# DigitalPhonetics/Intrinsic-Subgraph-Generation-for-VQA

Measured on AMD Instinct MI355X. Metric: GQA questions/sec, higher is better.
Workload: dtype f32

## Files before the change

### __graft_entry__.py

```python
from __future__ import annotations

import glob
import json
import os
import subprocess
import sys

ROOT = os.path.dirname(os.path.abspath(__file__))
PKG = os.path.join(ROOT, "intrinsic-subgraph-generation-for-vqa_amd")
CSRC = os.path.join(PKG, "csrc")
LIB = os.path.join(CSRC, "libisg_hip.so")
LOADER_LIB = os.path.join(CSRC, "libisg_loader.so")
if ROOT not in sys.path:
    sys.path.insert(0, ROOT)


HIP_FLAGS = ["-O3", "--offload-arch=gfx950", "-std=c++17", "-fPIC", "-Wall", "-Wno-unused-function",
             "-Werror=missing-field-initializers"]
EXTRA_FLAGS = {"isg_simple.hip": ["-fno-slp-vectorize"], "isg_mp_logits.hip": ["-fno-slp-vectorize"],
               "isg_sgenc_bwd.hip": ["-fno-slp-vectorize"]}


def flags_for(source: str):
    return HIP_FLAGS + EXTRA_FLAGS.get(os.path.basename(source), [])
# ... 2 lines not shown
def _stale(target: str, sources) -> bool:
    if not os.path.exists(target):
        return True
    t = os.path.getmtime(target)
    return any(os.path.getmtime(s) > t for s in sources)


def build(force: bool = False) -> None:
    sources = sorted(glob.glob(os.path.join(CSRC, "*.hip")))
    headers = glob.glob(os.path.join(CSRC, "*.hpp")) + [os.path.join(ROOT, "include", "isg.h"),
                                                        os.path.join(ROOT, "include", "isg_train.h"),
                                                        os.path.join(ROOT, "include", "isg_optim.h"),
                                                        os.path.join(ROOT, "include", "isg_fused.h"),
                                                        os.path.join(ROOT, "include", "isg_sgenc_train.h"),
                                                        os.path.join(ROOT, "include", "isg_dist.h"),
                                                        os.path.join(ROOT, "include", "isg_linear_train.h")]
    hipcc = os.environ.get("HIPCC", "/opt/rocm/bin/hipcc")
    flags = HIP_FLAGS
    objdir = os.path.join(CSRC, "_obj")
    os.makedirs(objdir, exist_ok=True)
    objs = [os.path.join(objdir, os.path.basename(s)[:-4] + ".o") for s in sources]
    stamp_path = LIB[:-3] + ".stamp"
    stamp = json.dumps({"sources": [os.path.basename(s) for s in sources], "flags": flags, "extra": EXTRA_FLAGS}, sort_keys=True)
    stamp_ok = os.path.exists(stamp_path) and open(stamp_path).read() == stamp
    relink = force or not stamp_ok
    if not force and stamp_ok and not _stale(LIB, sources + headers):
        todo = []
    else:
        old = json.loads(open(stamp_path).read()) if os.path.exists(stamp_path) else None
        flags_changed = old is not None and (old.get("flags") != flags or old.get("extra", {}) != EXTRA_FLAGS)
        todo = [(s, o) for s, o in zip(sources, objs) if force or flags_changed or _stale(o, [s] + headers)]
# ... 30 lines not shown
    _loader.load()
    lib = _lib.load()
    assert lib.isg_abi_version() == _lib.ABI_VERSION
    from isubgvqa_amd import _lib_train
    assert _lib_train.load().isg_train_abi_version() == _lib_train.ABI_VERSION
    from isubgvqa_amd import _lib_optim
    assert _lib_optim.load().isg_optim_abi_version() == _lib_optim.ABI_VERSION
    from isubgvqa_amd import _lib_fused
    assert _lib_fused.load().isg_fused_abi_version() == _lib_fused.ABI_VERSION
    from isubgvqa_amd import _lib_sgenc_train
    assert _lib_sgenc_train.load().isg_sgenc_train_abi_version() == _lib_sgenc_train.ABI_VERSION
    from isubgvqa_amd import _lib_dist
    assert _lib_dist.load().isg_dist_abi_version() == _lib_dist.ABI_VERSION
    from isubgvqa_amd import _lib_linear_train
    assert _lib_linear_train.load().isg_linear_train_abi_version() == _lib_linear_train.ABI_VERSION
    import isubgvqa_amd.models
    print(f"[build] ok: {LIB} ({os.path.getsize(LIB)} bytes), {len(_lib.SIGNATURES)} C-ABI symbols + "
          f"{len(_lib_train.SIGNATURES)} training + {len(_lib_optim.SIGNATURES)} optimizer + {len(_lib_fused.SIGNATURES)} fused-launch + "
          f"{len(_lib_sgenc_train.SIGNATURES)} scene-graph training + {len(_lib_dist.SIGNATURES)} data-parallel + "
          f"{len(_lib_linear_train.SIGNATURES)} Linear-backward entry points", flush=True)


STRICT_LIB = os.path.join(CSRC, "libisg_hip_strict.so")


def build_strict(sources, headers, objs, hipcc, relink: bool) -> None:
    objdir = os.path.join(CSRC, "_obj")
    strict = [s for s in sources if any(m in open(s).read() for m in ("ISG_WAIT(", "ISG_BARRIER("))]
    sobjs = {s: os.path.join(objdir, os.path.basename(s)[:-4] + ".strict.o") for s in strict}
    todo = [s for s in strict if relink or _stale(sobjs[s], [s] + headers)]
    if not todo and os.path.exists(STRICT_LIB) and not _stale(STRICT_LIB, sources + headers):
        return
    if any(not os.path.exists(o) for o in objs):
        if os.path.exists(STRICT_LIB):
            return
# ... 66 lines not shown
```

### intrinsic-subgraph-generation-for-vqa_amd/csrc/isg_layer_conv.hip

```cpp
#include "isg_f16x3.hpp"

#include "isg_diag.hpp"

ISG_DIAG_BUFFER(g_lc_stamps)
#define LC_STAMP(i) ISG_DIAG_ADD(i)

namespace isg {

typedef __attribute__((address_space(3))) void lc_lds_t;
typedef __attribute__((address_space(1))) void lc_glb_t;

constexpr int LC_ROWS = 64, LC_ECAP = 256, LC_C = 128, LC_K = 128, LC_LDX = LC_C + 4, LC_LDA = LC_K + 8, LC_THREADS = 512;
constexpr int LC_OFF_XR = LC_ROWS * LC_LDX * 4;
constexpr int LC_OFF_A = 2 * LC_ROWS * LC_LDX * 4;
constexpr int LC_OFF_TAB = LC_OFF_A + 2 * 64 * LC_LDA * 2;
constexpr int LC_OFF_RAW = LC_OFF_TAB + 2 * (LC_ECAP * 16 + LC_ECAP * 4 + 68 * 4) + LC_ECAP * 4 + 4 * 64 * 4 + 64 * 4 + 3 * LC_C * 4 +
                           4 * LC_C * 4;
constexpr int LC_OFF_LIVE = LC_OFF_RAW + LC_ROWS * LC_K * 4;
constexpr int LC_SMEM_BYTES = LC_OFF_LIVE + 2 * 4 * 8;
static_assert(LC_OFF_RAW % 16 == 0, "16-byte pieces");
static_assert(LC_SMEM_BYTES <= 160 * 1024, "one workgroup per CU");

struct LcArgs {
  const _Float16 *xp;
// ... 2 lines not shown
  const float *wn_inv, *bn;
  const _Float16 *ep;
  const float *ep_inv;
  const _Float16 *We;
  const float *we_inv, *att;
  const float *bias;
  const int *rowptr, *eid, *src, *dst, *ntiles;
  const int4 *tile_info;
  const float *edge_mask, *node_mask;
  float *out, *alpha;
  float *rowmax;
  int N, E, H, KSE, NTE, ldo;
  float slope;
  unsigned char *row_dead;
  int G;
};

struct LcLive {
  const unsigned long long *w;
  int p1, p2, p3, n;
};

__device__ __forceinline__ LcLive lc_live_load(const unsigned long long *sw) {
  int c[4];
#pragma unroll
  for (int i = 0; i < 4; ++i)
    c[i] = __builtin_amdgcn_readfirstlane(__popc((unsigned)sw[i]) + __popc((unsigned)(sw[i] >> 32)));
  return LcLive{sw, c[0], c[0] + c[1], c[0] + c[1] + c[2], c[0] + c[1] + c[2] + c[3]};
}

// ... 613 lines not shown
    LC_STAMP(6)
    if (!has_next) break;
    desc = desc_n;
    t = t_next;
    cur ^= 1;
  }
#undef LC_REQUEST_TILE
#undef LC_REQUEST_PLANES
#undef LC_REQUEST_MASKS
#undef LC_BALLOT
#undef LC_STORE_TILE
#undef LC_PLANES_LANDED
  ISG_DIAG_DUMP(g_lc_stamps, bid * 8 + wave, 12, )
}

constexpr int LG_MAXG = 6, LC_GROUP_DEFAULT = 4;
constexpr int LG_T_LG = LC_ECAP * 8, LG_T_SP = LG_T_LG + LC_ECAP * 4, LG_T_DR = LG_T_SP + LC_ECAP, LG_T_LV = LG_T_DR + LC_ECAP,
              LG_T_RP = LG_T_LV + LC_ECAP, LG_T_POS = LG_T_RP + 68 * 4, LG_TILE_BYTES = LG_T_POS + 64;
constexpr int LG_OFF_T = LC_OFF_A + 2 * 64 * LC_LDA * 2;
constexpr int LG_OFF_MISC = LG_OFF_T + LG_MAXG * LG_TILE_BYTES;
constexpr int LG_MISC_FLOATS = 4 * 64 + 3 * LC_C + 4 * LC_C + 64;
constexpr int LG_SMEM_BYTES = LG_OFF_MISC + LG_MISC_FLOATS * 4 + LG_MAXG * 16 + LG_MAXG * 8 + LG_MAXG * 4 * 8;
static_assert(LG_TILE_BYTES % 16 == 0 && LG_OFF_MISC % 16 == 0, "16-byte pieces");
static_assert(64 * 512 <= 2 * 64 * LC_LDA * 2, "the node planes fit the panel image they share LDS with");
static_assert(LG_SMEM_BYTES <= 160 * 1024, "one workgroup per CU");

template <int KSE_T, bool SL01>
__global__ __launch_bounds__(LC_THREADS, 2) void gatv2_layer_conv_groups_kernel(LcArgs a) {
  extern __shared__ __attribute__((aligned(16))) unsigned char lc_smem[];
  typedef float (*BufX)[LC_LDX];
  typedef _Float16 (*BufP)[64][LC_LDA];
  constexpr bool MASKED = true;
  BufX sXl = reinterpret_cast<BufX>(lc_smem);
  BufX sXr = reinterpret_cast<BufX>(lc_smem + LC_OFF_XR);
  BufP sA = reinterpret_cast<BufP>(lc_smem + LC_OFF_A);
  unsigned char *s_tiles = lc_smem + LG_OFF_T;
#define LG_EM(j) reinterpret_cast<int2 *>(s_tiles + (j) * LG_TILE_BYTES)
#define LG_LG(j) reinterpret_cast<float *>(s_tiles + (j) * LG_TILE_BYTES + LG_T_LG)
#define LG_SP(j) (s_tiles + (j) * LG_TILE_BYTES + LG_T_SP)
#define LG_DR(j) (s_tiles + (j) * LG_TILE_BYTES + LG_T_DR)
#define LG_LV(j) (s_tiles + (j) * LG_TILE_BYTES + LG_T_LV)
#define LG_RP(j) reinterpret_cast<int *>(s_tiles + (j) * LG_TILE_BYTES + LG_T_RP)
// ... 51 lines not shown
    s_bias[tid] = a.bias ? a.bias[hoff + tid] : 0.f;
    sXl[0][tid] = 0.f;
  } else if (tid < 3 * LC_C) {
    const int c = tid - LC_C;
    const int src_col = (c >> 7) * a.H * LC_C + hoff + (c & 127);
    s_bn[c] = a.bn[src_col];
    s_wninv[c] = a.wn_inv[src_col];
  }
  const float slope = a.slope;
  const int prow = half * 32 + fr;

#pragma unroll 1
  for (int tg = t; tg < T; tg += G * ngrp) {
    int tl = tid, ll = lane;
    asm volatile("" : "+v"(tl), "+v"(ll));
    int4 dsc[LG_MAXG];
    int ng = 0;
#pragma unroll
    for (int j = 0; j < LG_MAXG; ++j) {
      const int tj = tg + j * ngrp;
      const bool on = j < G && tj < T;
      const int4 d = a.tile_info[min(tj, T - 1)];
      dsc[j] = make_int4(on ? __builtin_amdgcn_readfirstlane(d.x) : 0, on ? min(__builtin_amdgcn_readfirstlane(d.y), LC_ROWS) : 0,
                         on ? __builtin_amdgcn_readfirstlane(d.z) : 0, on ? min(__builtin_amdgcn_readfirstlane(d.w), LC_ECAP) : 0);
      ng += on ? 1 : 0;
    }
    int srcv[LG_MAXG], eidv[LG_MAXG], dstv[LG_MAXG], rpv[LG_MAXG];
    float einvv[LG_MAXG], mskv[LG_MAXG];
#pragma unroll
    for (int j = 0; j < LG_MAXG; ++j) {
      srcv[j] = eidv[j] = dstv[j] = rpv[j] = 0;
      einvv[j] = 1.f;
      if (j < ng) {
        if (tl <= dsc[j].y) rpv[j] = a.rowptr[dsc[j].x + tl];
        if (tl < dsc[j].w) {
          srcv[j] = a.src[dsc[j].z + tl];
          eidv[j] = a.eid[dsc[j].z + tl];
          dstv[j] = a.dst[dsc[j].z + tl];
          einvv[j] = a.ep_inv[dsc[j].z + tl];
        }
      }
    }
    if (tl < LG_MAXG) s_touch[tl] = 0ull;
    __syncthreads();
#pragma unroll
    for (int j = 0; j < LG_MAXG; ++j) {
      mskv[j] = 1.f;
      if (j < ng && tl < dsc[j].w)
        mskv[j] = a.edge_mask ? a.edge_mask[eidv[j]] : a.node_mask[srcv[j]] * a.node_mask[dstv[j]];
    }
#pragma unroll
    for (int j = 0; j < LG_MAXG; ++j) {
      if (j < ng) {
        const int r0n = dsc[j].x, nrn = dsc[j].y, e0n = dsc[j].z, nen = dsc[j].w;
        if (tl <= nrn) LG_RP(j)[tl] = rpv[j] - e0n;
        if (tl == 0) s_desc[j] = dsc[j];
        if (tl < LC_ECAP) {
          const int sx = min(max(srcv[j] - r0n, 0), max(nrn - 1, 0));
          const int dz = min(max(dstv[j] - r0n, 0), max(nrn - 1, 0));
          const bool lv = tl < nen && (__float_as_int(mskv[j]) & 0x7fffffff) != 0;
          const unsigned long long bw = __ballot(lv);
          if (ll == 0) s_livew[j * 4 + wave] = bw;
          if (lv) atomicOr(&s_touch[j], (1ull << sx) | (1ull << dz));
          LG_EM(j)[tl] = make_int2(eidv[j], __float_as_int(mskv[j]));
          LG_LG(j)[tl] = lv ? einvv[j] : 0.f;
          LG_SP(j)[tl] = (unsigned char)sx;
          LG_DR(j)[tl] = (unsigned char)dz;
        }
      }
    }
    __syncthreads();
    LC_STAMP(0)

    int ntot = 0;
#pragma unroll
    for (int j = 0; j < LG_MAXG; ++j) ntot += j < ng ? __builtin_amdgcn_readfirstlane(__popcll(s_touch[j])) : 0;
    const int step = ntot <= LC_ROWS ? ng : 1;
#pragma unroll 1
    for (int ja = 0; ja < ng; ja += step) {
      const int jb = min(ja + step, ng);
      int cum[LG_MAXG];
      int nl = 0, nlive = 0;
#pragma unroll
      for (int j = 0; j < LG_MAXG; ++j) {
        if (j >= ja && j < jb) {
          const unsigned long long m = s_touch[j];
          if (tl < LC_ROWS) {
            const bool on = (m >> tl) & 1ull;
            const int p = nl + __popcll(m & ((1ull << tl) - 1ull));
            LG_POS(j)[tl] = (unsigned char)(on ? p : 0);
            if (on) s_nodes[p] = s_desc[j].x + tl;
          }
          int c[4];
#pragma unroll
          for (int i = 0; i < 4; ++i) {
            const unsigned long long w = s_livew[j * 4 + i];
            c[i] = __builtin_amdgcn_readfirstlane(__popc((unsigned)w) + __popc((unsigned)(w >> 32)));
          }
          if (tl < LC_ECAP) {
            const unsigned long long w = s_livew[j * 4 + wave];
            const int pre = (wave > 0 ? c[0] : 0) + (wave > 1 ? c[1] : 0) + (wave > 2 ? c[2] : 0);
            if ((w >> ll) & 1ull) LG_LV(j)[pre + __popcll(w & ((1ull << ll) - 1ull))] = (unsigned char)tl;
          }
          nl += __builtin_amdgcn_readfirstlane(__popcll(m));
          nlive += (c[0] + c[1]) + (c[2] + c[3]);
        }
        cum[j] = nlive;
      }
#define LG_FIND(k, jj, slot, e0v)                                                                                    \
  int jj = 0, slot, e0v;                                                                                             \
  {                                                                                                                  \
    int base_ = 0;                                                                                                   \
    _Pragma("unroll") for (int j_ = 0; j_ < LG_MAXG - 1; ++j_) {                                                     \
      const bool up_ = (k) >= cum[j_];                                                                               \
      jj += up_ ? 1 : 0;                                                                                             \
      base_ = up_ ? cum[j_] : base_;                                                                                 \
    }                                                                                                                \
// ... 189 lines not shown

extern "C" int isg_node_gate_planes(const uint16_t *x_planes, const float *x_inv_scale, const uint16_t *w_frag, const float *w_inv_scale,
                                    const float *b, const float *q, const int64_t *batch, int32_t double_index, float *gate,
                                    int64_t N, int32_t C, void *stream) {
  if (N < 0 || C <= 0) return ISG_EINVAL;
  auto mis = [](const void *p) { return (reinterpret_cast<uintptr_t>(p) & 15) != 0; };
  if (C != NG_C || mis(x_planes) || mis(w_inv_scale) || mis(b) || mis(q) || N >= (1ll << 31)) return ISG_EUNSUPPORTED;
  if (N == 0) return ISG_OK;
  if (!x_planes || !x_inv_scale || !w_frag || !w_inv_scale || !b || !q || !batch || !gate) return ISG_EINVAL;
  node_gate_planes_kernel<<<(unsigned)((N + NG_ROWS - 1) / NG_ROWS), 256, 0, as_stream(stream)>>>(
      reinterpret_cast<const _Float16 *>(x_planes), x_inv_scale, reinterpret_cast<const _Float16 *>(w_frag), w_inv_scale, b, q,
      reinterpret_cast<const long long *>(batch), double_index, gate, (int)N, sqrtf((float)C));
  return check_launch();
}

extern "C" int isg_gatv2_layer_conv(const uint16_t *x_planes, const float *x_inv_scale, const uint16_t *wn_frag, const float *wn_inv_scale,
                                    const float *bn, const uint16_t *edge_planes, const float *edge_inv_scale, const uint16_t *we_frag,
                                    const float *we_inv_scale, const float *att, const float *bias, const int32_t *rowptr,
                                    const int32_t *eid, const int32_t *src, const int32_t *dst, const int32_t *tile_info,
                                    const int32_t *ntiles, int64_t max_tiles, const float *node_mask, const float *edge_mask,
                                    float *out, int32_t ldo, float *alpha, float *rowmax, uint8_t *row_dead, int64_t N, int64_t E,
                                    int32_t H,
                                    int32_t C, int32_t K_in, int32_t K_edge, float negative_slope, void *stream) {
  if (N < 0 || E < 0 || H <= 0 || C <= 0 || K_in <= 0 || K_edge <= 0 || max_tiles < 0 || ldo < H * C) return ISG_EINVAL;
  auto mis = [](const void *p) { return (reinterpret_cast<uintptr_t>(p) & 15) != 0; };
  if (C != LC_C || K_in != LC_K || K_edge > LC_K || (K_edge & 3) != 0 || (ldo & 3) != 0 || H > 16 || mis(x_planes) ||
      mis(edge_planes) || mis(out) || (bias && mis(bias)) || mis(tile_info) || N >= (1ll << 31) || E >= (1ll << 31))
    return ISG_EUNSUPPORTED;
  if (N == 0 || max_tiles == 0) return ISG_OK;
  if (!x_planes || !x_inv_scale || !wn_frag || !wn_inv_scale || !bn ||
      (E > 0 && (!edge_planes || !edge_inv_scale || !eid || !src || !dst || !alpha)) || !we_frag || !we_inv_scale || !att || !rowptr ||
      !tile_info || !ntiles || !out)
    return ISG_EINVAL;
  static const bool dense_mask = [] { const char *e = getenv("ISG_LC_DENSE_MASK"); return e && atoi(e) != 0; }();
  LcArgs a = {
      .xp = reinterpret_cast<const _Float16 *>(x_planes), .xinv = x_inv_scale, .Wn = reinterpret_cast<const _Float16 *>(wn_frag),
      .wn_inv = wn_inv_scale, .bn = bn, .ep = reinterpret_cast<const _Float16 *>(edge_planes), .ep_inv = edge_inv_scale,
      .We = reinterpret_cast<const _Float16 *>(we_frag), .we_inv = we_inv_scale, .att = att, .bias = bias, .rowptr = rowptr,
      .eid = eid, .src = src, .dst = dst, .ntiles = ntiles, .tile_info = reinterpret_cast<const int4 *>(tile_info),
      .edge_mask = edge_mask, .node_mask = node_mask, .out = out, .alpha = alpha, .rowmax = rowmax, .N = (int)N, .E = (int)E,
      .H = H, .KSE = (K_edge + 15) / 16, .NTE = H * C / 32, .ldo = ldo, .slope = negative_slope, .row_dead = row_dead, .G = 1};
  if (!a.xp || !a.xinv || !a.Wn || !a.wn_inv || !a.bn || (a.E > 0 && (!a.ep || !a.ep_inv || !a.eid || !a.src || !a.dst || !a.alpha)) ||
      !a.We || !a.we_inv || !a.att || !a.rowptr || !a.tile_info || !a.ntiles || !a.out)
    return ISG_EINVAL;
  const int cus = device_cus();
  int gpx = (cus / 8) / H;
  if (gpx < 1) gpx = 1;
  const long long need = (max_tiles + 7) / 8;
  if (gpx > need) gpx = (int)need;
  const unsigned grid = 8u * (unsigned)H * (unsigned)gpx;
  hipStream_t st = as_stream(stream);
  static const int force_group = [] { const char *e = getenv("ISG_LC_GROUP"); return e ? atoi(e) : 0; }();
  {
    const long long tiles = std::max((N + LC_ROWS - 1) / LC_ROWS, (E + LC_ECAP - 1) / LC_ECAP);
    const long long per_wg = (std::min<long long>(tiles, max_tiles) + 8 * gpx - 1) / (8 * gpx);
    a.G = force_group > 0 ? std::min(force_group, LG_MAXG) : (int)std::max<long long>(1, std::min<long long>(LC_GROUP_DEFAULT, per_wg));
  }
#define LC_LAUNCH_G(KT, SL)                                                                                          \
  {                                                                                                                  \
    if (!dyn_lds_ok<&gatv2_layer_conv_groups_kernel<KT, SL>>(LG_SMEM_BYTES)) return ISG_EUNSUPPORTED;                \
    gatv2_layer_conv_groups_kernel<KT, SL><<<grid, LC_THREADS, LG_SMEM_BYTES, st>>>(a);                              \
  }
#define LC_LAUNCH(M, KT, SL, LV)                                                                                     \
  {                                                                                                                  \
    if (!dyn_lds_ok<&gatv2_layer_conv_kernel<M, KT, SL, LV>>(LC_SMEM_BYTES)) return ISG_EUNSUPPORTED;                \
    gatv2_layer_conv_kernel<M, KT, SL, LV><<<grid, LC_THREADS, LC_SMEM_BYTES, st>>>(a);                              \
  }
#define LC_LAUNCH_M(KT, SL)                                                                                          \
  {                                                                                                                  \
    if (dense_mask) LC_LAUNCH(true, KT, SL, false) else if (a.G > 1) LC_LAUNCH_G(KT, SL) else LC_LAUNCH(true, KT, SL, true) \
  }
  const bool masked = node_mask || edge_mask;
  const bool sl01 = negative_slope >= 0.f && negative_slope <= 1.f;
  if (a.KSE == 8 && sl01) {
    if (masked) LC_LAUNCH_M(8, true) else LC_LAUNCH(false, 8, true, false)
  } else if (sl01) {
    if (masked) LC_LAUNCH_M(0, true) else LC_LAUNCH(false, 0, true, false)
  } else {
    if (masked) LC_LAUNCH_M(0, false) else LC_LAUNCH(false, 0, false, false)
  }
#undef LC_LAUNCH_M
#undef LC_LAUNCH_G
#undef LC_LAUNCH
  return check_launch();
}

namespace isg {

constexpr int RO_ROWS = 64, RO_C = 128, RO_LDA = RO_C + 8, RO_LDC = RO_C + 4, RO_GPC = 128;
constexpr int RO_SMEM_BYTES = 2 * (2 * RO_ROWS * RO_LDA * 2) + (6 * 64 + RO_GPC + 4) * 4;
static_assert(RO_ROWS * RO_LDC * 4 <= 2 * RO_ROWS * RO_LDA * 2, "xn aliases the first plane image");

struct RoArgs {
  const float *x;
  const _Float16 *w1f, *w2f;
  const float *w1_inv, *b1, *w2_inv, *b2;
  const float *y_bound;
  const float *q;
  const float *node_mask;
// ... 258 lines not shown
```

### intrinsic-subgraph-generation-for-vqa_amd/ops.py

```python
from __future__ import annotations

import contextlib
import dataclasses
import operator
import sys
import types
import weakref
from dataclasses import dataclass, field
from typing import NamedTuple, Optional, Tuple

import torch
from torch import Tensor

from . import _lib

MAX_NODES_PER_GRAPH = 1024


@dataclasses.dataclass(frozen=True)
class Switches:
    plan_fused: bool = True
    bounds_to_host: bool = True
    mixed_dispatch: bool = True
    mixed_max_fraction: float = 0.12
# ... 1234 lines not shown
    if edge_attr.dtype != torch.float32:
        raise TypeError("gatv2_layer_conv: fp32 edge rows")
    cat_w = derived_weight("layer_conv_w", (lin_l.weight, lin_r.weight),
                           lambda: torch.cat([lin_l.weight.detach(), lin_r.weight.detach()], 0).contiguous())
    zeros = lambda m: torch.zeros(HC, dtype=torch.float32, device=dev) if m.bias is None else m.bias.detach()
    srcs = tuple(t for t in (lin_l.weight, lin_l.bias, lin_r.bias) if t is not None)
    cat_b = derived_weight("layer_conv_b", srcs, lambda: torch.cat([zeros(lin_l), zeros(lin_r)]).float().contiguous())
    wn, wn_inv = _weight_planes(cat_w, True, "f16x3")
    we, we_inv = _weight_planes(w_edge, True, "f16x3")
    (_, ntiles, cap, _), (ep, ep_inv) = plan.tiles_and_edge_planes(edge_attr, TILE_CONV_NODES, TILE_CONV_EDGES)
    shared, out, alpha, rowmax = _tile_conv_operands(plan, ntiles, cap, att, bias, node_mask, edge_mask, H, HC, want_rowmax, dev)
    row_dead = None
    if rowmax is not None and (node_mask is not None or edge_mask is not None):
        whole = plan.tile_mode(TILE_CONV_NODES, TILE_CONV_EDGES) == "tiles"
        row_dead = (torch.empty if whole else torch.zeros)(N, H, dtype=torch.uint8, device=dev)
    timer, ev1 = MP_TIMER, None
    if timer is not None:
        ev0, ev1 = timer.bracket({"N": N, "E": E, "H": H, "C": C, "K": K, "masked": node_mask is not None or edge_mask is not None,
                                  "feat_bytes": 4, "tile_conv": True, "layer_conv": True, "K_in": K_in})
        ev0.record()
    rc = lib.isg_gatv2_layer_conv(
        x.planes.data_ptr(), x.inv.data_ptr(), wn.data_ptr(), wn_inv.data_ptr(), cat_b.data_ptr(), ep.data_ptr(), ep_inv.data_ptr(),
        we.data_ptr(), we_inv.data_ptr(), *shared, 0 if row_dead is None else row_dead.data_ptr(), N, E, H, C, K_in, K,
        float(negative_slope), _stream())
    if not _launched(rc, "isg_gatv2_layer_conv", timer, ev1):
        return None
    sub = _mixed_sub(plan)
    if sub is not None:
        pl = x.planes.view(torch.float16).index_select(0, sub.nodes).float()
        xs = ((pl[:, 0] + pl[:, 1]) * x.inv.index_select(0, sub.nodes)[:, None]).contiguous()
        y = linear(xs, cat_w, cat_b)
        _oversize_conv(sub, y[:, :HC], y[:, HC:], edge_attr, w_edge, att, H, bias, node_mask, edge_mask, negative_slope,
                       out, alpha, rowmax)
    if rowmax is not None:
        attach_row_maxima(out, rowmax)
    if row_dead is not None:
        attach_dead_rows(out, row_dead)
    return out, alpha

# ... 1769 lines not shown
```

Measured before the change: 3.248 million.

## Precompute per-tile live-edge tables in a separate kernel for masked layer conv

Adds a pre-pass kernel that builds, for each tile, a 4 KiB image holding the edge ids, masks, scales, src/dst offsets, live-edge lists and row pointers. The grouped layer-conv kernel then loads these images straight into LDS with global_load_lds instead of gathering and computing them per group. The default group size also goes from 4 to 6 tiles. This takes the masked gather and compaction off the main kernel's critical path. In exchange it adds an extra launch, a temporary buffer allocation and extra global memory traffic.

```diff
diff --git a/__graft_entry__.py b/__graft_entry__.py
--- a/__graft_entry__.py
+++ b/__graft_entry__.py
@@ -40,7 +40,8 @@
                                                         os.path.join(ROOT, "include", "isg_fused.h"),
                                                         os.path.join(ROOT, "include", "isg_sgenc_train.h"),
                                                         os.path.join(ROOT, "include", "isg_dist.h"),
-                                                        os.path.join(ROOT, "include", "isg_linear_train.h")]
+                                                        os.path.join(ROOT, "include", "isg_linear_train.h"),
+                                                        os.path.join(ROOT, "include", "isg_masked.h")]
     hipcc = os.environ.get("HIPCC", "/opt/rocm/bin/hipcc")
     flags = HIP_FLAGS
     objdir = os.path.join(CSRC, "_obj")
@@ -101,11 +102,13 @@
     assert _lib_dist.load().isg_dist_abi_version() == _lib_dist.ABI_VERSION
     from isubgvqa_amd import _lib_linear_train
     assert _lib_linear_train.load().isg_linear_train_abi_version() == _lib_linear_train.ABI_VERSION
+    from isubgvqa_amd import _lib_masked
+    assert _lib_masked.load().isg_masked_abi_version() == _lib_masked.ABI_VERSION
     import isubgvqa_amd.models
     print(f"[build] ok: {LIB} ({os.path.getsize(LIB)} bytes), {len(_lib.SIGNATURES)} C-ABI symbols + "
           f"{len(_lib_train.SIGNATURES)} training + {len(_lib_optim.SIGNATURES)} optimizer + {len(_lib_fused.SIGNATURES)} fused-launch + "
           f"{len(_lib_sgenc_train.SIGNATURES)} scene-graph training + {len(_lib_dist.SIGNATURES)} data-parallel + "
-          f"{len(_lib_linear_train.SIGNATURES)} Linear-backward entry points", flush=True)
+          f"{len(_lib_linear_train.SIGNATURES)} Linear-backward + {len(_lib_masked.SIGNATURES)} masked-layer entry points", flush=True)
 
 
 STRICT_LIB = os.path.join(CSRC, "libisg_hip_strict.so")
diff --git a/include/isg_masked.h b/include/isg_masked.h
--- /dev/null
+++ b/include/isg_masked.h
@@ -0,0 +1,38 @@
+#ifndef ISG_MASKED_H
+#define ISG_MASKED_H
+
+#include <stdint.h>
+
+#ifdef __cplusplus
+extern "C" {
+#endif
+
+#define ISG_MASKED_ABI_VERSION 1
+
+int isg_masked_abi_version(void);
+
+#define ISG_LIVE_TABLES_TILE_BYTES 4176
+
+int64_t isg_layer_conv_live_tables_bytes(int64_t capacity);
+
+int isg_layer_conv_live_tables(const int32_t *rowptr, const int32_t *eid, const int32_t *src, const int32_t *dst,
+                               const float *edge_inv_scale, const int32_t *tile_info, const int32_t *ntiles, int64_t capacity,
+                               const float *node_mask, const float *edge_mask, uint8_t *tables, int64_t N, int64_t E, void *stream);
+
+int32_t isg_gatv2_layer_conv_group(int64_t N, int64_t E, int32_t H, int64_t max_tiles);
+
+int32_t isg_layer_conv_live_tables_enabled(void);
+
+int isg_gatv2_layer_conv_tables(const uint16_t *x_planes, const float *x_inv_scale, const uint16_t *wn_frag, const float *wn_inv_scale,
+                                const float *bn, const uint16_t *edge_planes, const float *edge_inv_scale, const uint16_t *we_frag,
+                                const float *we_inv_scale, const float *att, const float *bias, const int32_t *rowptr,
+                                const int32_t *eid, const int32_t *src, const int32_t *dst, const int32_t *tile_info,
+                                const int32_t *ntiles, int64_t max_tiles, const float *node_mask, const float *edge_mask,
+                                float *out, int32_t ldo, float *alpha, float *rowmax, uint8_t *row_dead, const uint8_t *live_tables,
+                                int64_t N, int64_t E, int32_t H, int32_t C, int32_t K_in, int32_t K_edge, float negative_slope,
+                                void *stream);
+
+#ifdef __cplusplus
+}
+#endif
+#endif
diff --git a/intrinsic-subgraph-generation-for-vqa_amd/_lib_masked.py b/intrinsic-subgraph-generation-for-vqa_amd/_lib_masked.py
--- /dev/null
+++ b/intrinsic-subgraph-generation-for-vqa_amd/_lib_masked.py
@@ -0,0 +1,28 @@
+from __future__ import annotations
+
+import ctypes
+import os
+
+from . import _lib
+
+HEADER_PATH = os.path.join(os.path.dirname(_lib._HERE), "include", "isg_masked.h")
+SIGNATURES, ABI_VERSION = _lib.read_header(HEADER_PATH)
+
+_bound = None
+
+
+def load():
+    global _bound
+    if _bound is not None:
+        return _bound
+    _lib.load()
+    lib = ctypes.CDLL(_lib.LIB_PATH)
+    try:
+        _lib.bind(lib, SIGNATURES)
+    except AttributeError as e:
+        raise _lib.IsgError(f"{_lib.LIB_PATH} lacks a symbol of include/isg_masked.h ({e}): rebuild it (build())") from None
+    v = lib.isg_masked_abi_version()
+    if v != ABI_VERSION:
+        raise _lib.IsgError(f"libisg_hip.so masked-layer ABI version {v}, binding expects {ABI_VERSION}")
+    _bound = lib
+    return lib
diff --git a/intrinsic-subgraph-generation-for-vqa_amd/csrc/isg_layer_conv.hip b/intrinsic-subgraph-generation-for-vqa_amd/csrc/isg_layer_conv.hip
--- a/intrinsic-subgraph-generation-for-vqa_amd/csrc/isg_layer_conv.hip
+++ b/intrinsic-subgraph-generation-for-vqa_amd/csrc/isg_layer_conv.hip
@@ -1,6 +1,8 @@
 #include "isg_f16x3.hpp"
 
 #include "isg_diag.hpp"
+#include "isg_live_tables.hpp"
+#include "../../include/isg_masked.h"
 
 ISG_DIAG_BUFFER(g_lc_stamps)
 #define LC_STAMP(i) ISG_DIAG_ADD(i)
@@ -40,6 +42,7 @@
   float slope;
   unsigned char *row_dead;
   int G;
+  const unsigned char *live_tables;
 };
 
 struct LcLive {
@@ -683,18 +686,19 @@
   ISG_DIAG_DUMP(g_lc_stamps, bid * 8 + wave, 12, )
 }
 
-constexpr int LG_MAXG = 6, LC_GROUP_DEFAULT = 4;
-constexpr int LG_T_LG = LC_ECAP * 8, LG_T_SP = LG_T_LG + LC_ECAP * 4, LG_T_DR = LG_T_SP + LC_ECAP, LG_T_LV = LG_T_DR + LC_ECAP,
-              LG_T_RP = LG_T_LV + LC_ECAP, LG_T_POS = LG_T_RP + 68 * 4, LG_TILE_BYTES = LG_T_POS + 64;
+constexpr int LG_MAXG = 6, LC_GROUP_DEFAULT = 6;
+static_assert(LT_ROWS == LC_ROWS && LT_ECAP == LC_ECAP, "the table sets are cut for this kernel's tiles");
 constexpr int LG_OFF_T = LC_OFF_A + 2 * 64 * LC_LDA * 2;
 constexpr int LG_OFF_MISC = LG_OFF_T + LG_MAXG * LG_TILE_BYTES;
 constexpr int LG_MISC_FLOATS = 4 * 64 + 3 * LC_C + 4 * LC_C + 64;
 constexpr int LG_SMEM_BYTES = LG_OFF_MISC + LG_MISC_FLOATS * 4 + LG_MAXG * 16 + LG_MAXG * 8 + LG_MAXG * 4 * 8;
-static_assert(LG_TILE_BYTES % 16 == 0 && LG_OFF_MISC % 16 == 0, "16-byte pieces");
+static_assert(LG_TILE_BYTES % 16 == 0 && LG_OFF_T % 16 == 0 && LG_OFF_MISC % 16 == 0 && LG_T_RP + 64 * 4 == 4 * 1024 &&
+                  LG_TILE_BYTES == 4 * 1024 + 5 * 16 && LG_H_DESC == 4096 + 16 && LG_H_TOUCH == 4096 + 32 && LG_H_LIVE == 4096 + 48,
+              "16-byte pieces; the fetch of a table set from memory: four 1 KiB pieces, then five 16-byte ones");
 static_assert(64 * 512 <= 2 * 64 * LC_LDA * 2, "the node planes fit the panel image they share LDS with");
 static_assert(LG_SMEM_BYTES <= 160 * 1024, "one workgroup per CU");
 
-template <int KSE_T, bool SL01>
+template <int KSE_T, bool SL01, bool TABLES>
 __global__ __launch_bounds__(LC_THREADS, 2) void gatv2_layer_conv_groups_kernel(LcArgs a) {
   extern __shared__ __attribute__((aligned(16))) unsigned char lc_smem[];
   typedef float (*BufX)[LC_LDX];
@@ -776,62 +780,93 @@
   for (int tg = t; tg < T; tg += G * ngrp) {
     int tl = tid, ll = lane;
     asm volatile("" : "+v"(tl), "+v"(ll));
-    int4 dsc[LG_MAXG];
     int ng = 0;
-#pragma unroll
-    for (int j = 0; j < LG_MAXG; ++j) {
-      const int tj = tg + j * ngrp;
-      const bool on = j < G && tj < T;
-      const int4 d = a.tile_info[min(tj, T - 1)];
-      dsc[j] = make_int4(on ? __builtin_amdgcn_readfirstlane(d.x) : 0, on ? min(__builtin_amdgcn_readfirstlane(d.y), LC_ROWS) : 0,
-                         on ? __builtin_amdgcn_readfirstlane(d.z) : 0, on ? min(__builtin_amdgcn_readfirstlane(d.w), LC_ECAP) : 0);
-      ng += on ? 1 : 0;
-    }
-    int srcv[LG_MAXG], eidv[LG_MAXG], dstv[LG_MAXG], rpv[LG_MAXG];
-    float einvv[LG_MAXG], mskv[LG_MAXG];
-#pragma unroll
-    for (int j = 0; j < LG_MAXG; ++j) {
-      srcv[j] = eidv[j] = dstv[j] = rpv[j] = 0;
-      einvv[j] = 1.f;
-      if (j < ng) {
-        if (tl <= dsc[j].y) rpv[j] = a.rowptr[dsc[j].x + tl];
-        if (tl < dsc[j].w) {
-          srcv[j] = a.src[dsc[j].z + tl];
-          eidv[j] = a.eid[dsc[j].z + tl];
-          dstv[j] = a.dst[dsc[j].z + tl];
-          einvv[j] = a.ep_inv[dsc[j].z + tl];
+    if constexpr (TABLES) {
+#pragma unroll
+      for (int j = 0; j < LG_MAXG; ++j) ng += j < G && tg + j * ngrp < T ? 1 : 0;
+      __syncthreads();
+#pragma unroll 1
+      for (int u = wave; u < 4 * ng; u += LC_THREADS / 64) {
+        const int j = u >> 2, pc = u & 3;
+        const unsigned char *img = a.live_tables + (size_t)(tg + j * ngrp) * LG_TILE_BYTES;
+        __builtin_amdgcn_global_load_lds((lc_glb_t *)(img + pc * 1024 + ll * 16), (lc_lds_t *)(s_tiles + j * LG_TILE_BYTES + pc * 1024),
+                                         16, 0, 0);
+      }
+      if (tl < 5 * ng) {
+        const int j = tl / 5, pc = tl - 5 * j;
+        const uint4 v = *reinterpret_cast<const uint4 *>(a.live_tables + (size_t)(tg + j * ngrp) * LG_TILE_BYTES + 4096 + pc * 16);
+        const unsigned long long lo = (unsigned long long)v.x | ((unsigned long long)v.y << 32),
+                                 hi = (unsigned long long)v.z | ((unsigned long long)v.w << 32);
+        if (pc == 0) {
+          *reinterpret_cast<uint4 *>(s_tiles + j * LG_TILE_BYTES + 4096) = v;
+        } else if (pc == 1) {
+          s_desc[j] = make_int4((int)v.x, (int)v.y, (int)v.z, (int)v.w);
+        } else if (pc == 2) {
+          s_touch[j] = lo;
+        } else {
+          s_livew[j * 4 + 2 * (pc - 3)] = lo;
+          s_livew[j * 4 + 2 * (pc - 3) + 1] = hi;
         }
       }
-    }
-    if (tl < LG_MAXG) s_touch[tl] = 0ull;
-    __syncthreads();
-#pragma unroll
-    for (int j = 0; j < LG_MAXG; ++j) {
-      mskv[j] = 1.f;
-      if (j < ng && tl < dsc[j].w)
-        mskv[j] = a.edge_mask ? a.edge_mask[eidv[j]] : a.node_mask[srcv[j]] * a.node_mask[dstv[j]];
-    }
-#pragma unroll
-    for (int j = 0; j < LG_MAXG; ++j) {
-      if (j < ng) {
-        const int r0n = dsc[j].x, nrn = dsc[j].y, e0n = dsc[j].z, nen = dsc[j].w;
-        if (tl <= nrn) LG_RP(j)[tl] = rpv[j] - e0n;
-        if (tl == 0) s_desc[j] = dsc[j];
-        if (tl < LC_ECAP) {
-          const int sx = min(max(srcv[j] - r0n, 0), max(nrn - 1, 0));
-          const int dz = min(max(dstv[j] - r0n, 0), max(nrn - 1, 0));
-          const bool lv = tl < nen && (__float_as_int(mskv[j]) & 0x7fffffff) != 0;
-          const unsigned long long bw = __ballot(lv);
-          if (ll == 0) s_livew[j * 4 + wave] = bw;
-          if (lv) atomicOr(&s_touch[j], (1ull << sx) | (1ull << dz));
-          LG_EM(j)[tl] = make_int2(eidv[j], __float_as_int(mskv[j]));
-          LG_LG(j)[tl] = lv ? einvv[j] : 0.f;
-          LG_SP(j)[tl] = (unsigned char)sx;
-          LG_DR(j)[tl] = (unsigned char)dz;
+      ISG_WAIT(0x0F70);
+      __syncthreads();
+    } else {
+      int4 dsc[LG_MAXG];
+#pragma unroll
+      for (int j = 0; j < LG_MAXG; ++j) {
+        const int tj = tg + j * ngrp;
+        const bool on = j < G && tj < T;
+        const int4 d = a.tile_info[min(tj, T - 1)];
+        dsc[j] = make_int4(on ? __builtin_amdgcn_readfirstlane(d.x) : 0, on ? min(__builtin_amdgcn_readfirstlane(d.y), LC_ROWS) : 0,
+                           on ? __builtin_amdgcn_readfirstlane(d.z) : 0, on ? min(__builtin_amdgcn_readfirstlane(d.w), LC_ECAP) : 0);
+        ng += on ? 1 : 0;
+      }
+      int srcv[LG_MAXG], eidv[LG_MAXG], dstv[LG_MAXG], rpv[LG_MAXG];
+      float einvv[LG_MAXG], mskv[LG_MAXG];
+#pragma unroll
+      for (int j = 0; j < LG_MAXG; ++j) {
+        srcv[j] = eidv[j] = dstv[j] = rpv[j] = 0;
+        einvv[j] = 1.f;
+        if (j < ng) {
+          if (tl <= dsc[j].y) rpv[j] = a.rowptr[dsc[j].x + tl];
+          if (tl < dsc[j].w) {
+            srcv[j] = a.src[dsc[j].z + tl];
+            eidv[j] = a.eid[dsc[j].z + tl];
+            dstv[j] = a.dst[dsc[j].z + tl];
+            einvv[j] = a.ep_inv[dsc[j].z + tl];
+          }
         }
       }
-    }
-    __syncthreads();
+      if (tl < LG_MAXG) s_touch[tl] = 0ull;
+      __syncthreads();
+#pragma unroll
+      for (int j = 0; j < LG_MAXG; ++j) {
+        mskv[j] = 1.f;
+        if (j < ng && tl < dsc[j].w)
+          mskv[j] = a.edge_mask ? a.edge_mask[eidv[j]] : a.node_mask[srcv[j]] * a.node_mask[dstv[j]];
+      }
+#pragma unroll
+      for (int j = 0; j < LG_MAXG; ++j) {
+        if (j < ng) {
+          const int r0n = dsc[j].x, nrn = dsc[j].y, e0n = dsc[j].z, nen = dsc[j].w;
+          if (tl <= nrn) LG_RP(j)[tl] = rpv[j] - e0n;
+          if (tl == 0) s_desc[j] = dsc[j];
+          if (tl < LC_ECAP) {
+            const int sx = min(max(srcv[j] - r0n, 0), max(nrn - 1, 0));
+            const int dz = min(max(dstv[j] - r0n, 0), max(nrn - 1, 0));
+            const bool lv = tl < nen && (__float_as_int(mskv[j]) & 0x7fffffff) != 0;
+            const unsigned long long bw = __ballot(lv);
+            if (ll == 0) s_livew[j * 4 + wave] = bw;
+            if (lv) atomicOr(&s_touch[j], (1ull << sx) | (1ull << dz));
+            LG_EM(j)[tl] = make_int2(eidv[j], __float_as_int(mskv[j]));
+            LG_LG(j)[tl] = lv ? einvv[j] : 0.f;
+            LG_SP(j)[tl] = (unsigned char)sx;
+            LG_DR(j)[tl] = (unsigned char)dz;
+          }
+        }
+      }
+      __syncthreads();
+    }
     LC_STAMP(0)
 
     int ntot = 0;
@@ -859,10 +894,12 @@
             const unsigned long long w = s_livew[j * 4 + i];
             c[i] = __builtin_amdgcn_readfirstlane(__popc((unsigned)w) + __popc((unsigned)(w >> 32)));
           }
-          if (tl < LC_ECAP) {
-            const unsigned long long w = s_livew[j * 4 + wave];
-            const int pre = (wave > 0 ? c[0] : 0) + (wave > 1 ? c[1] : 0) + (wave > 2 ? c[2] : 0);
-            if ((w >> ll) & 1ull) LG_LV(j)[pre + __popcll(w & ((1ull << ll) - 1ull))] = (unsigned char)tl;
+          if constexpr (!TABLES) {
+            if (tl < LC_ECAP) {
+              const unsigned long long w = s_livew[j * 4 + wave];
+              const int pre = (wave > 0 ? c[0] : 0) + (wave > 1 ? c[1] : 0) + (wave > 2 ? c[2] : 0);
+              if ((w >> ll) & 1ull) LG_LV(j)[pre + __popcll(w & ((1ull << ll) - 1ull))] = (unsigned char)tl;
+            }
           }
           nl += __builtin_amdgcn_readfirstlane(__popcll(m));
           nlive += (c[0] + c[1]) + (c[2] + c[3]);
@@ -1082,6 +1119,89 @@
   return check_launch();
 }
 
+static int lc_group_rule(int64_t N, int64_t E, int32_t H, int64_t max_tiles, int *gpx_out) {
+  static const int force_group = [] { const char *e = getenv("ISG_LC_GROUP"); return e ? atoi(e) : 0; }();
+  const int cus = device_cus();
+  int gpx = (cus / 8) / H;
+  if (gpx < 1) gpx = 1;
+  const long long need = (max_tiles + 7) / 8;
+  if (gpx > need) gpx = (int)need;
+  if (gpx < 1) gpx = 1;
+  if (gpx_out) *gpx_out = gpx;
+  const long long tiles = std::max((N + LC_ROWS - 1) / LC_ROWS, (E + LC_ECAP - 1) / LC_ECAP);
+  const long long per_wg = (std::min<long long>(tiles, max_tiles) + 8 * gpx - 1) / (8 * gpx);
+  return force_group > 0 ? std::min(force_group, LG_MAXG) : (int)std::max<long long>(1, std::min<long long>(LC_GROUP_DEFAULT, per_wg));
+}
+
+static int lc_launch(const uint16_t *x_planes, const float *x_inv_scale, const uint16_t *wn_frag, const float *wn_inv_scale,
+                     const float *bn, const uint16_t *edge_planes, const float *edge_inv_scale, const uint16_t *we_frag,
+                     const float *we_inv_scale, const float *att, const float *bias, const int32_t *rowptr, const int32_t *eid,
+                     const int32_t *src, const int32_t *dst, const int32_t *tile_info, const int32_t *ntiles, int64_t max_tiles,
+                     const float *node_mask, const float *edge_mask, float *out, int32_t ldo, float *alpha, float *rowmax,
+                     uint8_t *row_dead, const uint8_t *live_tables, int64_t N, int64_t E, int32_t H, int32_t C, int32_t K_in,
+                     int32_t K_edge, float negative_slope, void *stream) {
+  if (N < 0 || E < 0 || H <= 0 || C <= 0 || K_in <= 0 || K_edge <= 0 || max_tiles < 0 || ldo < H * C) return ISG_EINVAL;
+  auto mis = [](const void *p) { return (reinterpret_cast<uintptr_t>(p) & 15) != 0; };
+  if (C != LC_C || K_in != LC_K || K_edge > LC_K || (K_edge & 3) != 0 || (ldo & 3) != 0 || H > 16 || mis(x_planes) ||
+      mis(edge_planes) || mis(out) || (bias && mis(bias)) || mis(tile_info) || mis(live_tables) || N >= (1ll << 31) ||
+      E >= (1ll << 31))
+    return ISG_EUNSUPPORTED;
+  if (N == 0 || max_tiles == 0) return ISG_OK;
+  if (!x_planes || !x_inv_scale || !wn_frag || !wn_inv_scale || !bn ||
+      (E > 0 && (!edge_planes || !edge_inv_scale || !eid || !src || !dst || !alpha)) || !we_frag || !we_inv_scale || !att || !rowptr ||
+      !tile_info || !ntiles || !out)
+    return ISG_EINVAL;
+  static const bool dense_mask = [] { const char *e = getenv("ISG_LC_DENSE_MASK"); return e && atoi(e) != 0; }();
+  if (!isg_layer_conv_live_tables_enabled()) live_tables = nullptr;
+  LcArgs a = {
+      .xp = reinterpret_cast<const _Float16 *>(x_planes), .xinv = x_inv_scale, .Wn = reinterpret_cast<const _Float16 *>(wn_frag),
+      .wn_inv = wn_inv_scale, .bn = bn, .ep = reinterpret_cast<const _Float16 *>(edge_planes), .ep_inv = edge_inv_scale,
+      .We = reinterpret_cast<const _Float16 *>(we_frag), .we_inv = we_inv_scale, .att = att, .bias = bias, .rowptr = rowptr,
+      .eid = eid, .src = src, .dst = dst, .ntiles = ntiles, .tile_info = reinterpret_cast<const int4 *>(tile_info),
+      .edge_mask = edge_mask, .node_mask = node_mask, .out = out, .alpha = alpha, .rowmax = rowmax, .N = (int)N, .E = (int)E,
+      .H = H, .KSE = (K_edge + 15) / 16, .NTE = H * C / 32, .ldo = ldo, .slope = negative_slope, .row_dead = row_dead, .G = 1,
+      .live_tables = live_tables};
+  if (!a.xp || !a.xinv || !a.Wn || !a.wn_inv || !a.bn || (a.E > 0 && (!a.ep || !a.ep_inv || !a.eid || !a.src || !a.dst || !a.alpha)) ||
+      !a.We || !a.we_inv || !a.att || !a.rowptr || !a.tile_info || !a.ntiles || !a.out)
+    return ISG_EINVAL;
+  int gpx = 1;
+  a.G = lc_group_rule(N, E, H, max_tiles, &gpx);
+  const unsigned grid = 8u * (unsigned)H * (unsigned)gpx;
+  hipStream_t st = as_stream(stream);
+#define LC_LAUNCH_GT(KT, SL, TB)                                                                                     \
+  {                                                                                                                  \
+    if (!dyn_lds_ok<&gatv2_layer_conv_groups_kernel<KT, SL, TB>>(LG_SMEM_BYTES)) return ISG_EUNSUPPORTED;            \
+    gatv2_layer_conv_groups_kernel<KT, SL, TB><<<grid, LC_THREADS, LG_SMEM_BYTES, st>>>(a);                          \
+  }
+#define LC_LAUNCH_G(KT, SL)                                                                                          \
+  {                                                                                                                  \
+    if (a.live_tables) LC_LAUNCH_GT(KT, SL, true) else LC_LAUNCH_GT(KT, SL, false)                                   \
+  }
+#define LC_LAUNCH(M, KT, SL, LV)                                                                                     \
+  {                                                                                                                  \
+    if (!dyn_lds_ok<&gatv2_layer_conv_kernel<M, KT, SL, LV>>(LC_SMEM_BYTES)) return ISG_EUNSUPPORTED;                \
+    gatv2_layer_conv_kernel<M, KT, SL, LV><<<grid, LC_THREADS, LC_SMEM_BYTES, st>>>(a);                              \
+  }
+#define LC_LAUNCH_M(KT, SL)                                                                                          \
+  {                                                                                                                  \
+    if (dense_mask) LC_LAUNCH(true, KT, SL, false) else if (a.G > 1) LC_LAUNCH_G(KT, SL) else LC_LAUNCH(true, KT, SL, true) \
+  }
+  const bool masked = node_mask || edge_mask;
+  const bool sl01 = negative_slope >= 0.f && negative_slope <= 1.f;
+  if (a.KSE == 8 && sl01) {
+    if (masked) LC_LAUNCH_M(8, true) else LC_LAUNCH(false, 8, true, false)
+  } else if (sl01) {
+    if (masked) LC_LAUNCH_M(0, true) else LC_LAUNCH(false, 0, true, false)
+  } else {
+    if (masked) LC_LAUNCH_M(0, false) else LC_LAUNCH(false, 0, false, false)
+  }
+#undef LC_LAUNCH_M
+#undef LC_LAUNCH_G
+#undef LC_LAUNCH_GT
+#undef LC_LAUNCH
+  return check_launch();
+}
+
 extern "C" int isg_gatv2_layer_conv(const uint16_t *x_planes, const float *x_inv_scale, const uint16_t *wn_frag, const float *wn_inv_scale,
                                     const float *bn, const uint16_t *edge_planes, const float *edge_inv_scale, const uint16_t *we_frag,
                                     const float *we_inv_scale, const float *att, const float *bias, const int32_t *rowptr,
@@ -1090,67 +1210,33 @@
                                     float *out, int32_t ldo, float *alpha, float *rowmax, uint8_t *row_dead, int64_t N, int64_t E,
                                     int32_t H,
                                     int32_t C, int32_t K_in, int32_t K_edge, float negative_slope, void *stream) {
-  if (N < 0 || E < 0 || H <= 0 || C <= 0 || K_in <= 0 || K_edge <= 0 || max_tiles < 0 || ldo < H * C) return ISG_EINVAL;
-  auto mis = [](const void *p) { return (reinterpret_cast<uintptr_t>(p) & 15) != 0; };
-  if (C != LC_C || K_in != LC_K || K_edge > LC_K || (K_edge & 3) != 0 || (ldo & 3) != 0 || H > 16 || mis(x_planes) ||
-      mis(edge_planes) || mis(out) || (bias && mis(bias)) || mis(tile_info) || N >= (1ll << 31) || E >= (1ll << 31))
-    return ISG_EUNSUPPORTED;
-  if (N == 0 || max_tiles == 0) return ISG_OK;
-  if (!x_planes || !x_inv_scale || !wn_frag || !wn_inv_scale || !bn ||
-      (E > 0 && (!edge_planes || !edge_inv_scale || !eid || !src || !dst || !alpha)) || !we_frag || !we_inv_scale || !att || !rowptr ||
-      !tile_info || !ntiles || !out)
-    return ISG_EINVAL;
-  static const bool dense_mask = [] { const char *e = getenv("ISG_LC_DENSE_MASK"); return e && atoi(e) != 0; }();
-  LcArgs a = {
-      .xp = reinterpret_cast<const _Float16 *>(x_planes), .xinv = x_inv_scale, .Wn = reinterpret_cast<const _Float16 *>(wn_frag),
-      .wn_inv = wn_inv_scale, .bn = bn, .ep = reinterpret_cast<const _Float16 *>(edge_planes), .ep_inv = edge_inv_scale,
-      .We = reinterpret_cast<const _Float16 *>(we_frag), .we_inv = we_inv_scale, .att = att, .bias = bias, .rowptr = rowptr,
-      .eid = eid, .src = src, .dst = dst, .ntiles = ntiles, .tile_info = reinterpret_cast<const int4 *>(tile_info),
-      .edge_mask = edge_mask, .node_mask = node_mask, .out = out, .alpha = alpha, .rowmax = rowmax, .N = (int)N, .E = (int)E,
-      .H = H, .KSE = (K_edge + 15) / 16, .NTE = H * C / 32, .ldo = ldo, .slope = negative_slope, .row_dead = row_dead, .G = 1};
-  if (!a.xp || !a.xinv || !a.Wn || !a.wn_inv || !a.bn || (a.E > 0 && (!a.ep || !a.ep_inv || !a.eid || !a.src || !a.dst || !a.alpha)) ||
-      !a.We || !a.we_inv || !a.att || !a.rowptr || !a.tile_info || !a.ntiles || !a.out)
-    return ISG_EINVAL;
-  const int cus = device_cus();
-  int gpx = (cus / 8) / H;
-  if (gpx < 1) gpx = 1;
-  const long long need = (max_tiles + 7) / 8;
-  if (gpx > need) gpx = (int)need;
-  const unsigned grid = 8u * (unsigned)H * (unsigned)gpx;
-  hipStream_t st = as_stream(stream);
-  static const int force_group = [] { const char *e = getenv("ISG_LC_GROUP"); return e ? atoi(e) : 0; }();
-  {
-    const long long tiles = std::max((N + LC_ROWS - 1) / LC_ROWS, (E + LC_ECAP - 1) / LC_ECAP);
-    const long long per_wg = (std::min<long long>(tiles, max_tiles) + 8 * gpx - 1) / (8 * gpx);
-    a.G = force_group > 0 ? std::min(force_group, LG_MAXG) : (int)std::max<long long>(1, std::min<long long>(LC_GROUP_DEFAULT, per_wg));
-  }
-#define LC_LAUNCH_G(KT, SL)                                                                                          \
-  {                                                                                                                  \
-    if (!dyn_lds_ok<&gatv2_layer_conv_groups_kernel<KT, SL>>(LG_SMEM_BYTES)) return ISG_EUNSUPPORTED;                \
-    gatv2_layer_conv_groups_kernel<KT, SL><<<grid, LC_THREADS, LG_SMEM_BYTES, st>>>(a);                              \
-  }
-#define LC_LAUNCH(M, KT, SL, LV)                                                                                     \
-  {                                                                                                                  \
-    if (!dyn_lds_ok<&gatv2_layer_conv_kernel<M, KT, SL, LV>>(LC_SMEM_BYTES)) return ISG_EUNSUPPORTED;                \
-    gatv2_layer_conv_kernel<M, KT, SL, LV><<<grid, LC_THREADS, LC_SMEM_BYTES, st>>>(a);                              \
-  }
-#define LC_LAUNCH_M(KT, SL)                                                                                          \
-  {                                                                                                                  \
-    if (dense_mask) LC_LAUNCH(true, KT, SL, false) else if (a.G > 1) LC_LAUNCH_G(KT, SL) else LC_LAUNCH(true, KT, SL, true) \
-  }
-  const bool masked = node_mask || edge_mask;
-  const bool sl01 = negative_slope >= 0.f && negative_slope <= 1.f;
-  if (a.KSE == 8 && sl01) {
-    if (masked) LC_LAUNCH_M(8, true) else LC_LAUNCH(false, 8, true, false)
-  } else if (sl01) {
-    if (masked) LC_LAUNCH_M(0, true) else LC_LAUNCH(false, 0, true, false)
-  } else {
-    if (masked) LC_LAUNCH_M(0, false) else LC_LAUNCH(false, 0, false, false)
-  }
-#undef LC_LAUNCH_M
-#undef LC_LAUNCH_G
-#undef LC_LAUNCH
-  return check_launch();
+  return lc_launch(x_planes, x_inv_scale, wn_frag, wn_inv_scale, bn, edge_planes, edge_inv_scale, we_frag, we_inv_scale, att, bias,
+                   rowptr, eid, src, dst, tile_info, ntiles, max_tiles, node_mask, edge_mask, out, ldo, alpha, rowmax, row_dead,
+                   nullptr, N, E, H, C, K_in, K_edge, negative_slope, stream);
+}
+
+extern "C" int isg_gatv2_layer_conv_tables(const uint16_t *x_planes, const float *x_inv_scale, const uint16_t *wn_frag,
+                                           const float *wn_inv_scale, const float *bn, const uint16_t *edge_planes,
+                                           const float *edge_inv_scale, const uint16_t *we_frag, const float *we_inv_scale,
+                                           const float *att, const float *bias, const int32_t *rowptr, const int32_t *eid,
+                                           const int32_t *src, const int32_t *dst, const int32_t *tile_info, const int32_t *ntiles,
+                                           int64_t max_tiles, const float *node_mask, const float *edge_mask, float *out, int32_t ldo,
+                                           float *alpha, float *rowmax, uint8_t *row_dead, const uint8_t *live_tables, int64_t N,
+                                           int64_t E, int32_t H, int32_t C, int32_t K_in, int32_t K_edge, float negative_slope,
+                                           void *stream) {
+  return lc_launch(x_planes, x_inv_scale, wn_frag, wn_inv_scale, bn, edge_planes, edge_inv_scale, we_frag, we_inv_scale, att, bias,
+                   rowptr, eid, src, dst, tile_info, ntiles, max_tiles, node_mask, edge_mask, out, ldo, alpha, rowmax, row_dead,
+                   live_tables, N, E, H, C, K_in, K_edge, negative_slope, stream);
+}
+
+extern "C" int32_t isg_gatv2_layer_conv_group(int64_t N, int64_t E, int32_t H, int64_t max_tiles) {
+  if (N <= 0 || E < 0 || H <= 0 || H > 16 || max_tiles <= 0) return 1;
+  return lc_group_rule(N, E, H, max_tiles, nullptr);
+}
+
+extern "C" int32_t isg_layer_conv_live_tables_enabled(void) {
+  static const bool on = [] { const char *e = getenv("ISG_LC_TABLES"); return !e || atoi(e) != 0; }();
+  return on ? 1 : 0;
 }
 
 namespace isg {
diff --git a/intrinsic-subgraph-generation-for-vqa_amd/csrc/isg_live_tables.hip b/intrinsic-subgraph-generation-for-vqa_amd/csrc/isg_live_tables.hip
--- /dev/null
+++ b/intrinsic-subgraph-generation-for-vqa_amd/csrc/isg_live_tables.hip
@@ -0,0 +1,95 @@
+#include "isg_common.hpp"
+#include "isg_live_tables.hpp"
+#include "../../include/isg_masked.h"
+
+namespace isg {
+
+static_assert(LG_TILE_BYTES == ISG_LIVE_TABLES_TILE_BYTES, "include/isg_masked.h states the image size");
+
+struct LtArgs {
+  const int *rowptr, *eid, *src, *dst, *ntiles;
+  const float *ep_inv;
+  const int4 *tile_info;
+  const float *node_mask;
+  const float *edge_mask;
+  unsigned char *tables;
+  int N, E;
+};
+
+__global__ __launch_bounds__(LT_ECAP) void layer_conv_live_tables_kernel(LtArgs a) {
+  __shared__ __attribute__((aligned(16))) unsigned char s_img[LG_TILE_BYTES];
+  __shared__ unsigned long long s_touch, s_livew[4];
+  const int t = blockIdx.x;
+  if (t >= *a.ntiles) return;
+  const int tl = threadIdx.x, ll = tl & 63, wave = tl >> 6;
+  const int4 d = a.tile_info[t];
+  const int r0n = d.x, nrn = min(d.y, LT_ROWS), e0n = d.z, nen = min(d.w, LT_ECAP);
+  for (int i = tl; i < LG_TILE_BYTES / 16; i += LT_ECAP) reinterpret_cast<uint4 *>(s_img)[i] = make_uint4(0u, 0u, 0u, 0u);
+  if (tl == 0) s_touch = 0ull;
+  int srcv = 0, eidv = 0, dstv = 0, rpv = 0;
+  float einv = 1.f, msk = 1.f;
+  if (tl <= nrn && r0n >= 0 && r0n + tl <= a.N) rpv = a.rowptr[r0n + tl];
+  const bool in = tl < nen && e0n >= 0 && e0n + tl < a.E;
+  if (in) {
+    srcv = a.src[e0n + tl];
+    eidv = a.eid[e0n + tl];
+    dstv = a.dst[e0n + tl];
+    einv = a.ep_inv[e0n + tl];
+    if (a.edge_mask)
+      msk = a.edge_mask[min(max(eidv, 0), a.E - 1)];
+    else
+      msk = a.node_mask[min(max(srcv, 0), a.N - 1)] * a.node_mask[min(max(dstv, 0), a.N - 1)];
+  }
+  __syncthreads();
+  if (tl <= nrn) reinterpret_cast<int *>(s_img + LG_T_RP)[tl] = rpv - e0n;
+  const int sx = min(max(srcv - r0n, 0), max(nrn - 1, 0));
+  const int dz = min(max(dstv - r0n, 0), max(nrn - 1, 0));
+  const bool lv = tl < nen && (__float_as_int(msk) & 0x7fffffff) != 0;
+  const unsigned long long bw = __ballot(lv);
+  if (ll == 0) s_livew[wave] = bw;
+  if (lv) atomicOr(&s_touch, (1ull << sx) | (1ull << dz));
+  reinterpret_cast<int2 *>(s_img)[tl] = make_int2(eidv, __float_as_int(msk));
+  reinterpret_cast<float *>(s_img + LG_T_LG)[tl] = lv ? einv : 0.f;
+  s_img[LG_T_SP + tl] = (unsigned char)sx;
+  s_img[LG_T_DR + tl] = (unsigned char)dz;
+  __syncthreads();
+  int pre = 0;
+  for (int i = 0; i < wave; ++i) pre += __popcll(s_livew[i]);
+  if (lv) s_img[LG_T_LV + pre + __popcll(bw & ((1ull << ll) - 1ull))] = (unsigned char)tl;
+  if (tl == 0) {
+    *reinterpret_cast<int4 *>(s_img + LG_H_DESC) = make_int4(r0n, nrn, e0n, nen);
+    *reinterpret_cast<unsigned long long *>(s_img + LG_H_TOUCH) = s_touch;
+  }
+  if (tl < 4) reinterpret_cast<unsigned long long *>(s_img + LG_H_LIVE)[tl] = s_livew[tl];
+  __syncthreads();
+  uint4 *dst = reinterpret_cast<uint4 *>(a.tables + (size_t)t * LG_TILE_BYTES);
+  for (int i = tl; i < LG_TILE_BYTES / 16; i += LT_ECAP) dst[i] = reinterpret_cast<const uint4 *>(s_img)[i];
+}
+
+}
+
+using namespace isg;
+
+extern "C" int isg_masked_abi_version(void) { return ISG_MASKED_ABI_VERSION; }
+
+extern "C" int64_t isg_layer_conv_live_tables_bytes(int64_t capacity) { return capacity > 0 ? capacity * (int64_t)LG_TILE_BYTES : 0; }
+
+extern "C" int isg_layer_conv_live_tables(const int32_t *rowptr, const int32_t *eid, const int32_t *src, const int32_t *dst,
+                                          const float *edge_inv_scale, const int32_t *tile_info, const int32_t *ntiles,
+                                          int64_t capacity, const float *node_mask, const float *edge_mask, uint8_t *tables,
+                                          int64_t N, int64_t E, void *stream) {
+  if (N < 0 || E < 0 || capacity < 0) return ISG_EINVAL;
+  auto mis = [](const void *p) { return (reinterpret_cast<uintptr_t>(p) & 15) != 0; };
+  if (mis(tables) || mis(tile_info) || N >= (1ll << 31) || E >= (1ll << 31) || capacity >= (1ll << 31)) return ISG_EUNSUPPORTED;
+  if (N == 0 || capacity == 0) return ISG_OK;
+  if (!node_mask && !edge_mask) return ISG_EINVAL;
+  if (E > 0 && (!eid || !src || !dst || !edge_inv_scale)) return ISG_EINVAL;
+  LtArgs a = {.rowptr = rowptr, .eid = eid, .src = src, .dst = dst, .ntiles = ntiles, .ep_inv = edge_inv_scale,
+              .tile_info = reinterpret_cast<const int4 *>(tile_info), .node_mask = node_mask, .edge_mask = edge_mask,
+              .tables = tables, .N = (int)N, .E = (int)E};
+  if (!a.rowptr || (a.E > 0 && (!a.eid || !a.src || !a.dst || !a.ep_inv)) || !a.ntiles || !a.tile_info || !a.tables ||
+      (!a.node_mask && !a.edge_mask))
+    return ISG_EINVAL;
+  layer_conv_live_tables_kernel<<<(unsigned)capacity, LT_ECAP, 0, as_stream(stream)>>>(a);
+  return check_launch();
+}
diff --git a/intrinsic-subgraph-generation-for-vqa_amd/csrc/isg_live_tables.hpp b/intrinsic-subgraph-generation-for-vqa_amd/csrc/isg_live_tables.hpp
--- /dev/null
+++ b/intrinsic-subgraph-generation-for-vqa_amd/csrc/isg_live_tables.hpp
@@ -0,0 +1,19 @@
+#pragma once
+
+namespace isg {
+
+constexpr int LT_ROWS = 64, LT_ECAP = 256;
+constexpr int LG_T_LG = LT_ECAP * 8;
+constexpr int LG_T_SP = LG_T_LG + LT_ECAP * 4;
+constexpr int LG_T_DR = LG_T_SP + LT_ECAP;
+constexpr int LG_T_LV = LG_T_DR + LT_ECAP;
+constexpr int LG_T_RP = LG_T_LV + LT_ECAP;
+constexpr int LG_T_POS = LG_T_RP + 68 * 4;
+constexpr int LG_TILE_BYTES = LG_T_POS + 64;
+constexpr int LG_H_DESC = LG_T_POS;
+constexpr int LG_H_TOUCH = LG_T_POS + 16;
+constexpr int LG_H_LIVE = LG_T_POS + 32;
+static_assert(LG_TILE_BYTES % 16 == 0 && LG_T_RP % 16 == 0 && LG_T_POS % 16 == 0, "16-byte pieces");
+static_assert(LG_TILE_BYTES == 4176 && LG_H_LIVE + 32 == LG_TILE_BYTES, "the image layout include/isg_masked.h documents");
+
+}
diff --git a/intrinsic-subgraph-generation-for-vqa_amd/ops.py b/intrinsic-subgraph-generation-for-vqa_amd/ops.py
--- a/intrinsic-subgraph-generation-for-vqa_amd/ops.py
+++ b/intrinsic-subgraph-generation-for-vqa_amd/ops.py
@@ -1272,15 +1272,26 @@
     if rowmax is not None and (node_mask is not None or edge_mask is not None):
         whole = plan.tile_mode(TILE_CONV_NODES, TILE_CONV_EDGES) == "tiles"
         row_dead = (torch.empty if whole else torch.zeros)(N, H, dtype=torch.uint8, device=dev)
+    mlib, tables = None, None
+    if (node_mask is not None or edge_mask is not None) and cap > 0:
+        from . import _lib_masked
+        mlib = _lib_masked.load()
+        if mlib.isg_layer_conv_live_tables_enabled() and mlib.isg_gatv2_layer_conv_group(N, E, H, cap) > 1:
+            tables = torch.empty(mlib.isg_layer_conv_live_tables_bytes(cap), dtype=torch.uint8, device=dev)
     timer, ev1 = MP_TIMER, None
     if timer is not None:
         ev0, ev1 = timer.bracket({"N": N, "E": E, "H": H, "C": C, "K": K, "masked": node_mask is not None or edge_mask is not None,
                                   "feat_bytes": 4, "tile_conv": True, "layer_conv": True, "K_in": K_in})
         ev0.record()
-    rc = lib.isg_gatv2_layer_conv(
-        x.planes.data_ptr(), x.inv.data_ptr(), wn.data_ptr(), wn_inv.data_ptr(), cat_b.data_ptr(), ep.data_ptr(), ep_inv.data_ptr(),
-        we.data_ptr(), we_inv.data_ptr(), *shared, 0 if row_dead is None else row_dead.data_ptr(), N, E, H, C, K_in, K,
-        float(negative_slope), _stream())
+    front = (x.planes.data_ptr(), x.inv.data_ptr(), wn.data_ptr(), wn_inv.data_ptr(), cat_b.data_ptr(), ep.data_ptr(), ep_inv.data_ptr(),
+             we.data_ptr(), we_inv.data_ptr(), *shared, 0 if row_dead is None else row_dead.data_ptr())
+    if tables is None:
+        rc = lib.isg_gatv2_layer_conv(*front, N, E, H, C, K_in, K, float(negative_slope), _stream())
+    else:
+        _, _, rowptr_p, eid_p, src_p, dst_p, tile_info_p, ntiles_p, _, nm_p, em_p = shared[:11]
+        _lib.check(mlib.isg_layer_conv_live_tables(rowptr_p, eid_p, src_p, dst_p, ep_inv.data_ptr(), tile_info_p, ntiles_p, cap,
+                                                   nm_p, em_p, tables.data_ptr(), N, E, _stream()), "isg_layer_conv_live_tables")
+        rc = mlib.isg_gatv2_layer_conv_tables(*front, tables.data_ptr(), N, E, H, C, K_in, K, float(negative_slope), _stream())
     if not _launched(rc, "isg_gatv2_layer_conv", timer, ev1):
         return None
     sub = _mixed_sub(plan)
```

Result: faster. 3.307 million (median of 6 runs) (+1.8%).
